# gyhandy/Neural-Sim-NeRF

Hardware: AMD Instinct MI355X
Metric: Mray-samples/sec at 400x400, 64+128 samples, 8x256 MLP (higher is better)
Workload: dtype f16x2

## Files before the change

### neural_sim_nerf_amd/csrc/nsr_kernels.hip

```cpp
#include <hip/hip_runtime.h>
#include <stdint.h>
#include "nsr_device.h"

#if !defined(NSR_UNIT_F32) && !defined(NSR_UNIT_H2) && !defined(NSR_UNIT_B3) && !defined(NSR_UNIT_X16)
#define NSR_UNIT_F32 1
#define NSR_UNIT_H2 1
#define NSR_UNIT_B3 1
#define NSR_UNIT_X16 1
#endif
#ifndef NSR_UNIT_F32
#define NSR_UNIT_F32 0
#endif
#ifndef NSR_UNIT_H2
#define NSR_UNIT_H2 0
#endif
#ifndef NSR_UNIT_B3
#define NSR_UNIT_B3 0
#endif
#ifndef NSR_UNIT_X16
#define NSR_UNIT_X16 0
#endif
#define NSR_CAT_(a, b) a##b
#define NSR_CAT(a, b) NSR_CAT_(a, b)

// ... 208 lines not shown
constexpr int kMlpH2 = 2;

template <int NMO>
__device__ __forceinline__ uint4 relu_mask(const f32x16 (&acc)[NMO]) {
  unsigned w[4] = {0u, 0u, 0u, 0u};
#pragma unroll
  for (int mo = 0; mo < NMO; ++mo)
#pragma unroll
    for (int r = 0; r < 16; ++r) {
      const int on = max(__float_as_int(acc[mo][r]), 0) - 1;
      w[mo >> 1] = __builtin_amdgcn_alignbit(w[mo >> 1], (unsigned)on, 31);
    }
  return make_uint4(w[0], w[1], w[2], w[3]);
}

__device__ __forceinline__ float enc_trig(float a, int k) {
  const double kMagic = 6755399441055744.0;
  const double t = (double)a * 0.63661977236758134308;
  const double tm = t + kMagic;
  const int n = __double2loint(tm) + k;
  const double f = t - (tm - kMagic);
  const float r = (float)(f * 1.57079632679489661923);
  const float z = r * r;
  float ps = __builtin_fmaf(-1.9515295891e-4f, z, 8.3321608736e-3f);
  ps = __builtin_fmaf(ps, z, -1.6666654611e-1f);
  ps = __builtin_fmaf(ps * z, r, r);
  float pc = __builtin_fmaf(2.443315711809948e-5f, z, -1.388731625493765e-3f);
  pc = __builtin_fmaf(pc, z, 4.166664568298827e-2f);
  pc = __builtin_fmaf(pc * z, z, __builtin_fmaf(-0.5f, z, 1.0f));
  const float v = (n & 1) ? pc : ps;
  return __uint_as_float(__float_as_uint(v) ^ ((unsigned)(n & 2) << 30));
}

__device__ __forceinline__ float enc_domain(float x, int nfreq) {
  return __builtin_fabsf(x) < ldexpf(1.0f, 25 - nfreq) ? x : __builtin_nanf("");
}

__device__ __forceinline__ float enc_poison(float px, float py, float pz, float vx, float vy, float vz) {
  const float a = (enc_domain(px, kMultires) * 0.0f + enc_domain(py, kMultires) * 0.0f) + enc_domain(pz, kMultires) * 0.0f;
  const float b = (enc_domain(vx, kMultiresViews) * 0.0f + enc_domain(vy, kMultiresViews) * 0.0f) +
                  enc_domain(vz, kMultiresViews) * 0.0f;
  return __builtin_fabsf(a + b);
}

template <bool CAPTURE, int MODE = kMlpF32>
__device__ __forceinline__ void mlp_pass(Ring& rg, const float* aux, f32x4 (&A0)[4], f32x4 (&A1)[4], int lane,
                                         float px, float py, float pz, float vx, float vy, float vz,
                                         float (&raw)[4], uint4* mask_dst = nullptr , int mask_tid = 0,
                                         long long* tp = nullptr ) {
#ifdef NSR_PHASE_TIMING
  long long tpl = clock64();
#define NSR_TP(i) do { if (tp) { const long long t_ = clock64(); tp[i] += t_ - tpl; tpl = t_; } } while (0)
#else
#define NSR_TP(i) do { } while (0)
#endif
  const int h = lane >> 5;
  const int h4 = aux_half(lane);
  const float poison = enc_poison(px, py, pz, vx, vy, vz);
  float e[32];
  float ed[16];
  {
    const float p[3] = {px, py, pz};
    const float v[3] = {vx, vy, vz};
#pragma unroll
    for (int L = 0; L < kMultires; ++L)
#pragma unroll
      for (int ax = 0; ax < 3; ++ax) e[3 * L + ax] = enc_trig(enc_domain(p[ax], kMultires) * (float)(1 << L), h);
#pragma unroll
    for (int L = 0; L < kMultiresViews; ++L)
#pragma unroll
      for (int ax = 0; ax < 3; ++ax) ed[3 * L + ax] = enc_trig(enc_domain(v[ax], kMultiresViews) * (float)(1 << L), h);
    e[30] = h ? pz : px;
    e[31] = h ? 0.0f : py;
    ed[12] = h ? vz : vx;
    ed[13] = h ? 0.0f : vy;
    ed[14] = 0.0f;
    ed[15] = 0.0f;
  }

  f32x16 acc[8];
  f32x16 in[8];
  auto enc_src = [&](int kb, int i) { return e[(8 * kb + i) & 31]; };
  auto in_src = [&](int kb, int i) { return in[(kb >> 1) & 7][8 * (kb & 1) + i]; };
  constexpr bool B3 = MODE == kMlpB3;
  constexpr bool H2M = MODE == kMlpH2;
  float amax = 0.0f;
  const float* h2s = aux + kAuxH2Scale;
#if NSR_H2_SCHED == 3 && !defined(NSR_EXP_H2_NOFRAG) && !defined(NSR_EXP_H2_HALFBARRIER) && !defined(NSR_EXP_H2_NOSPLIT)
  constexpr bool TAIL = H2M && !CAPTURE;
#else
  constexpr bool TAIL = false;
#endif
  static_assert(kAuxBiasV == kAuxBias + 9 * 256, "the views layer's bias follows feature_linear's: 'bias of layer L + 1' for L = 8");
  NSR_TP(0);
  load_bias<8>(aux + kAuxBias, h4, acc);
  NSR_TP(2);
  if constexpr (B3) gemm_b3<8, 2>(rg, A0, A1, enc_src, acc, lane);
  else if constexpr (TAIL)
    gemm_h2_tail<4>(rg, A0, A1, enc_src, H2Scale{{h2s[0], 0.0f}, 4}, acc, lane, amax, H2Tail{acc, in, 0, h2_lds_base(aux + kAuxBias + 256, h4)});
  else if constexpr (H2M) gemm_h2<8, 4>(rg, A0, A1, enc_src, H2Scale{{h2s[0], 0.0f}, 4}, acc, lane, amax);
  else seg<8, 8>(rg, A0, A1, BArr<32>{e}, acc, lane);
  NSR_TP(1);
  if (CAPTURE) mask_dst[mask_tid] = relu_mask<8>(acc);
  if constexpr (!TAIL) {
#pragma unroll
    for (int mo = 0; mo < 8; ++mo) in[mo] = relu16(acc[mo]);
  }

  float alpha_part = 0.0f;
#pragma unroll 1
  for (int L = 1; L <= 8; ++L) {
    if constexpr (!TAIL) load_bias<8>(aux + kAuxBias + L * 256, h4, acc);
    NSR_TP(2);
    if (L == 5) {
      if constexpr (B3) gemm_b3<8, 2>(rg, A0, A1, enc_src, acc, lane);
      else if constexpr (H2M) gemm_h2<8, 4>(rg, A0, A1, enc_src, H2Scale{{h2s[9], 0.0f}, 4}, acc, lane, amax);
      else seg<8, 8>(rg, A0, A1, BArr<32>{e}, acc, lane);
      NSR_TP(1);
    }
    if (L == 8) {
      const float* wa = aux + kAuxWAlpha;
#pragma unroll
      for (int tq = 0; tq < 32; ++tq) {
        f32x4 w = *(const f32x4*)(wa + tq * 8 + h4);
#pragma unroll
        for (int kk = 0; kk < 4; ++kk)
          alpha_part = __builtin_fmaf(w[kk], in[(4 * tq + kk) >> 4][(4 * tq + kk) & 15], alpha_part);
      }
    }
    if constexpr (B3) gemm_b3<8, 8>(rg, A0, A1, in_src, acc, lane);
    else if constexpr (TAIL)
      gemm_h2_tail<16>(rg, A0, A1, in_src, H2Scale{{h2s[L], 0.0f}, 16}, acc, lane, amax,
                       H2Tail{acc, in, (L == 8) ? (int)0x80000000 : 0, h2_lds_base(aux + kAuxBias + (L + 1) * 256, h4)});
    else if constexpr (H2M) gemm_h2<8, 16>(rg, A0, A1, in_src, H2Scale{{h2s[L], 0.0f}, 16}, acc, lane, amax);
    else seg<8, 32>(rg, A0, A1, BRegs16<8>{in}, acc, lane);
    NSR_TP(1);
    if (CAPTURE && L < 8) mask_dst[L * 256 + mask_tid] = relu_mask<8>(acc);
    if constexpr (!TAIL) {
      const int thr = (L == 8) ? (int)0x80000000 : 0;
#pragma unroll
      for (int mo = 0; mo < 8; ++mo) in[mo] = clamp_bits16(acc[mo], thr);
    }
  }

  f32x16 av[4];
  if constexpr (TAIL) {
#pragma unroll
    for (int mo = 0; mo < 4; ++mo) av[mo] = acc[mo];
  } else {
    load_bias<4>(aux + kAuxBiasV, h4, av);
  }
  NSR_TP(2);
  if constexpr (B3) {
    auto v_src = [&](int kb, int i) {
      return kb < 16 ? in[(kb >> 1) & 7][8 * (kb & 1) + i] : (kb < 18 ? ed[(8 * (kb - 16) + i) & 15] : 0.0f);
    };
    gemm_b3<4, 5>(rg, A0, A1, v_src, av, lane);
  } else if constexpr (H2M) {
    auto v_src = [&](int kb, int i) { return kb < 16 ? in[(kb >> 1) & 7][8 * (kb & 1) + i] : ed[(8 * (kb - 16) + i) & 15]; };
    gemm_h2<4, 18>(rg, A0, A1, v_src, H2Scale{{h2s[10], h2s[11]}, 16}, av, lane, amax);
  } else {
    seg<4, 36>(rg, A0, A1, BViews{in, ed}, av, lane);
  }
  NSR_TP(1);
  if (CAPTURE) mask_dst[8 * 256 + mask_tid] = relu_mask<4>(av);

  float part[4] = {0.0f, 0.0f, 0.0f, alpha_part};
  if constexpr (H2M) {
    const float ov = amax > kH2Max ? __builtin_nanf("") : 0.0f;
    part[0] = part[1] = part[2] = ov;
    part[3] = alpha_part + ov;
  }
#pragma unroll
  for (int c = 0; c < 3; ++c) {
    const float* wr = aux + kAuxWRgb + c * 128;
#pragma unroll
    for (int mo = 0; mo < 4; ++mo)
#pragma unroll
      for (int rq = 0; rq < 4; ++rq) {
        f32x4 w = *(const f32x4*)(wr + (mo * 4 + rq) * 8 + h4);
#pragma unroll
        for (int ri = 0; ri < 4; ++ri)
          part[c] = __builtin_fmaf(w[ri], fmaxf(av[mo][rq * 4 + ri], 0.0f), part[c]);
      }
  }
#pragma unroll
  for (int c = 0; c < 4; ++c) {
    float other = __shfl_xor(part[c], 32);
    float lo_half = h ? other : part[c];
    float hi_half = h ? part[c] : other;
    raw[c] = ((lo_half + hi_half) + aux[(c < 3) ? (kAuxBRgb + c) : kAuxBAlpha]) + poison;
  }
  NSR_TP(3);
#undef NSR_TP
}

template <int NSS, int NFS>
struct ItemStateT {
  static constexpr int kNS = NSS, kNF = NFS;
  float tcoarse[NSS];
  float ufine[128];
  float ray[2][16];
  float zc[2][NSS];
  float rawc[2][NSS][4];
  float w0[2][NSS];
  float cdf[2][NSS];
  float zs[2][128];
  float zf[2][NFS];
  float rawf[2][NFS][4];
  float alpha[2][NFS];
  float wf[2][NFS];
  float tf[2][NFS];
  float om[2][NFS];
  float bwd_scratch[2][NFS][2];
  float psum[2][NFS / 32][12];
  float gnorm[2];
  float res[2][8];
};
typedef ItemStateT<64, 192> ItemState;
typedef ItemStateT<128, 256> ItemStateBig;
static_assert(sizeof(ItemState) == 23048, "the YCB-V layout is part of the shipped kernels' LDS budget");
template <int NS> struct ItemStateFor { typedef ItemState type; };
template <> struct ItemStateFor<128> { typedef ItemStateBig type; };

__device__ __forceinline__ float sigmoidf_(float x) { return 1.0f / (1.0f + expf(-x)); }

template <int S, int R = 2, int STRIDE = S, typename ST>
__device__ __forceinline__ void composite(ST& st, const float* z, float* raw, float* wout, float* tout, int tid,
                                          const float* noise = nullptr ,
                                          long long row0 = 0, int valid = R) {
  static_assert(S % 8 == 0, "scan is unrolled by 8");
  for (int idx = tid; idx < R * S; idx += 256) {
    const int r = idx / S, i = idx - r * S;
    const float* zr = z + r * STRIDE;
    float dist = (i < S - 1) ? (zr[i + 1] - zr[i]) : 1e10f;
    dist = dist * st.ray[r][11];
    float* q = raw + (r * STRIDE + i) * 4;
    if (noise) q[3] = q[3] + noise[(row0 + (r < valid ? r : 0)) * S + i];
    const float sigma = fmaxf(q[3], 0.0f);
    const float a = 1.0f - expf(-sigma * dist);
    st.alpha[r][i] = a;
    st.om[r][i] = (1.0f - a) + 1e-10f;
    q[0] = sigmoidf_(q[0]);
    q[1] = sigmoidf_(q[1]);
    q[2] = sigmoidf_(q[2]);
  }
  __syncthreads();
  if ((tid & 63) == 0 && tid < 64 * R) {
    const int r = tid >> 6;
    double T = 1.0;
#pragma unroll 1
    for (int i0 = 0; i0 < S; i0 += 8) {
      double f[8];
#pragma unroll
// ... 356 lines not shown
  unsigned ovf_cap;
  const unsigned long long* item_list;
  const unsigned* item_count;
  unsigned item_cap;
};

__device__ __forceinline__ void load_aux(char* smem, const RenderArgs& a, int tid) {
  float* dst = (float*)(smem + kLdsAux);
  for (int i = tid; i < kAuxFloats; i += 256) {
    dst[i] = a.aux[0][i];
    dst[kAuxFloats + i] = a.aux[1][i];
  }
}

#if NSR_UNIT_F32
__global__ void k_set_args(const RenderArgs a, RenderArgs* dst) {
  *dst = a;
  *a.work_counter = 0ull;
  if (a.ovf_stat) a.ovf_stat[0] = 0u;
  if (a.epoch_counter) dst->epoch = *a.epoch_counter = *a.epoch_counter % 4094u + 1u;
}
#endif

constexpr long long kItemMask = (1ll << 62) - 1;
__device__ __forceinline__ long long queue_next_item(const RenderArgs& q) {
  const unsigned long long v = atomicAdd(q.work_counter, 1ull);
  if (q.item_list) {
    unsigned n = *q.item_count;
    n = n < q.item_cap ? n : q.item_cap;
    return v < (unsigned long long)n ? (long long)q.item_list[v] : -1ll;
  }
  return v < (unsigned long long)((q.n_rays + 1) >> 1) ? (long long)(v | (3ull << 62)) : -1ll;
}
__device__ __forceinline__ long long queue_items(const RenderArgs& q) {
  if (q.item_list) { const unsigned n = *q.item_count; return (long long)(n < q.item_cap ? n : q.item_cap); }
  return (q.n_rays + 1) >> 1;
}
__device__ __forceinline__ void range_mark(int* ovf, float chk, int lane) {
#ifndef NSR_EXP_NO_RANGE
  if (chk != chk && lane < 32) atomicAdd(ovf, 1);
#endif
}
__device__ __forceinline__ unsigned range_report(const RenderArgs& a, int* ovf, long long item, int valid) {
#ifdef NSR_EXP_NO_RANGE
  return 0u;
#endif
  const int p0 = ovf[0], p1 = valid == 2 ? ovf[1] : 0;
  if ((p0 | p1) != 0 && a.ovf_stat) {
    const unsigned long long mask = (p0 ? 1ull : 0ull) | (p1 ? 2ull : 0ull);
    const unsigned n = atomicAdd(a.ovf_stat, 1u);
    atomicAdd(a.ovf_stat + 1, (unsigned)(p0 + p1));
    if (n < a.ovf_cap) {
      a.ovf_items[n] = (unsigned long long)item | (mask << 62);
      atomicAdd(a.ovf_stat + 2, (unsigned)((p0 != 0) + (p1 != 0)));
    } else {
      atomicAdd(a.ovf_stat + 3, 1u);
      return (unsigned)mask;
    }
  }
  return 0u;
}
__device__ __forceinline__ void range_poison(const RenderArgs& a, long long ray0, unsigned mask) {
  const float qn = __builtin_nanf("");
  for (int r = 0; r < 2; ++r) {
    if (!((mask >> r) & 1u)) continue;
    const long long rr = ray0 + r;
    float* const v3[2] = {a.rgb, a.rgb0};
    float* const v1[5] = {a.disp, a.acc, a.disp0, a.acc0, a.z_std};
    for (int k = 0; k < 2; ++k) if (v3[k]) { v3[k][rr * 3] = qn; v3[k][rr * 3 + 1] = qn; v3[k][rr * 3 + 2] = qn; }
    for (int k = 0; k < 5; ++k) if (v1[k]) v1[k][rr] = qn;
  }
}

#ifdef NSR_PHASE_TIMING
#define NSR_T(i) do { if (threadIdx.x == 0) { const long long t_ = clock64(); tacc[i] += t_ - tlast; tlast = t_; } } while (0)
#else
#define NSR_T(i) do { } while (0)
#endif

template <int MODE, int NI = 128, int NS = 64>
__device__ __forceinline__ void render32_body(const RenderArgs* __restrict__ ap, char* smem) {
  constexpr bool B3 = MODE == kMlpB3;
  constexpr int NF = NS + NI;
  constexpr int NP = (2 * NF + 127) / 128;
  constexpr int NPC = (2 * NS + 127) / 128;
  constexpr int LNS = NS == 32 ? 5 : (NS == 64 ? 6 : 7);
  typedef typename ItemStateFor<NS>::type ST;
  static_assert((NS == 32 || NS == 64 || NS == 128) && NF % 32 == 0 && NS <= ST::kNS && NF <= ST::kNF,
                "a wave's points belong to one ray; the item state holds kNS coarse / kNF fine samples per ray");
  const RenderArgs& a_setup = *ap;
#ifdef NSR_PHASE_TIMING
  long long tacc[8] = {0, 0, 0, 0, 0, 0, 0, 0};
  long long tpass[4] = {0, 0, 0, 0};
  long long tlast = clock64();
#define NSR_TPASS tpass
#else
#define NSR_TPASS nullptr
#endif
  const int tid0 = threadIdx.x;
  const int lane = tid0 & 63;
  const int wave = __builtin_amdgcn_readfirstlane(tid0 >> 6);
  const int j = lane & 31;
  ST& st = *(ST*)(smem + kLdsState);

  const long long n_rays = a_setup.n_rays;
  if ((long long)blockIdx.x >= queue_items(a_setup)) return;
  const int fine = a_setup.fine;
  int* ovf = (int*)&st.ray[1][14];

  Ring rg;
  ring_init(rg, smem, a_setup.nets, a_setup.net_stride, fine ? NPC + NP : NPC, wave, lane);
  rg.pn0 = NPC; rg.pn1 = NPC + NP;

  f32x4 A0[4], A1[4];
  if constexpr (B3) ring_start<kRingSlots, kStreamSlabsB3, kStreamSlabsB3Bwd>(rg, A0, lane);
  else if constexpr (MODE == kMlpH2) ring_start<kRingSlots, kStreamSlabs, kStreamSlabs, kH2RingLag>(rg, A0, lane);
  else ring_start(rg, A0, lane);

  load_aux(smem, a_setup, tid0);
  if (tid0 < NS) st.tcoarse[tid0] = a_setup.tcoarse[tid0];
  if (tid0 < NI) st.ufine[tid0] = a_setup.ufine[tid0];
  __syncthreads();
  const float* aux_c = (const float*)(smem + kLdsAux);

  long long* item_slot = (long long*)&st.ray[0][14];
  auto next_item = [&]() -> long long {
    if (opaque_v(tid0) == 0) *item_slot = queue_next_item(*opaque_s(ap));
    __syncthreads();
    const long long v = uniform64(*item_slot);
    __syncthreads();
    return v;
  };
  long long packed = next_item();
  int pass = 0;
#pragma unroll 1
  while (packed != -1ll) {
    const long long item = packed & kItemMask;
    const long long ray0 = item * 2;
    const int valid = (ray0 + 1 < n_rays) ? 2 : 1;
    const int wmask = (int)((unsigned long long)packed >> 62) & (valid == 2 ? 3 : 1);
    auto wr = [&](int r) { return ((wmask >> r) & 1) != 0; };
    if (pass == 0) {
      const RenderArgs& a = *opaque_s(ap);
      const int tid = opaque_v(tid0);
      const float near_ = a.near_, far_ = a.far_;
      if (tid < 2) {
        const long long rr = ray0 + (tid < valid ? tid : 0);
        float o[3], d[3];
        if (a.camera) {
          const long long hw = (long long)a.H * a.W;
          const long long v = rr / hw;
          const int pix = (int)(rr - v * hw);
          gen_ray(a.c2w + v * 12, a.fx, a.fy, a.cx, a.cy, pix / a.W, pix % a.W, o, d);
        } else {
#pragma unroll
          for (int c = 0; c < 3; ++c) { o[c] = a.rays_o[rr * 3 + c]; d[c] = a.rays_d[rr * 3 + c]; }
        }
        const float nrm = sqrtf(((d[0] * d[0]) + (d[1] * d[1])) + (d[2] * d[2]));
        const float* vd = a.camera ? nullptr : a.viewdirs;
#pragma unroll
        for (int c = 0; c < 3; ++c) {
          st.ray[tid][c] = o[c]; st.ray[tid][3 + c] = d[c];
          st.ray[tid][6 + c] = vd ? vd[rr * 3 + c] : d[c] / nrm;
        }
        st.ray[tid][9] = a.near_rays ? a.near_rays[rr] : near_;
        st.ray[tid][10] = a.near_rays ? a.far_rays[rr] : far_;
        st.ray[tid][11] = nrm;
        st.ray[tid][12] = a.white_bkgd ? 1.0f : 0.0f;
      }
      if (MODE == kMlpH2 && (tid == 64 || tid == 65)) ovf[tid - 64] = 0;
      if (tid < 2 * NS) {
        const int r = tid >> LNS, i = tid & (NS - 1);
        const float t = st.tcoarse[i];
        const long long rb = ray0 + (r < valid ? r : 0);
        st.zc[r][i] = coarse_z(a.near_rays ? a.near_rays[rb] : near_, a.near_rays ? a.far_rays[rb] : far_, t, a.lindisp);
      }
      __syncthreads();
      if (a.t_rand) perturb_coarse_z<NS>(st, a.t_rand, ray0, valid, tid);
      NSR_T(0);
    }

    {
      int r, i;
      const float* zsrc;
      float* dst;
      bool real = true;
      if ((NPC == 1) ? (pass == 0) : (pass < NPC)) {
        if constexpr (NS == 64) {
          r = wave >> 1; i = 32 * (wave & 1) + j;
        } else {
          int q0 = 128 * pass + 32 * wave;
          if (2 * NS % 128 != 0 && q0 >= 2 * NS) { q0 = 2 * NS - 32; real = false; }
          r = q0 >> LNS; i = (q0 & (NS - 1)) + j;
        }
        zsrc = &st.zc[r][i]; dst = st.rawc[r][i];
      } else {
        int q0 = 128 * (pass - NPC) + 32 * wave;
        if (2 * NF % 128 != 0 && q0 >= 2 * NF) { q0 = 2 * NF - 32; real = false; }
        r = q0 / NF; i = q0 - r * NF + j;
        zsrc = &st.zf[r][i]; dst = st.rawf[r][i];
      }
      const float z = *zsrc;
      const float* ry = st.ray[r];
      float raw[4];
      mlp_pass<false, MODE>(rg, aux_c + (((NPC == 1) ? (pass == 0) : (pass < NPC)) ? 0 : kAuxFloats), A0, A1, lane, ry[0] + ry[3] * z, ry[1] + ry[4] * z,
               ry[2] + ry[5] * z, ry[6], ry[7], ry[8], raw, nullptr, 0, NSR_TPASS);
      if (lane < 32 && real) *(f32x4*)dst = f32x4{raw[0], raw[1], raw[2], raw[3]};
      if constexpr (MODE == kMlpH2) { if (real) range_mark(ovf + r, (raw[0] + raw[1]) + (raw[2] + raw[3]), lane); }
    }
    NSR_T(1);

    const RenderArgs& a = *opaque_s(ap);
    const int tid = opaque_v(tid0);
    if (NPC > 1 && pass < NPC - 1) {
      ++pass;
    } else if ((NPC == 1) ? (pass == 0) : (pass < NPC)) {
      __syncthreads();
      if (a.dbg_raw0) {
        if constexpr (NS == ST::kNS) {
          for (int idx = tid; idx < 2 * NS * 4; idx += 256) if (wr(idx >> (LNS + 2))) a.dbg_raw0[ray0 * (NS * 4) + idx] = (&st.rawc[0][0][0])[idx];
        } else {
          for (int idx = tid; idx < 2 * NS * 4; idx += 256)
            if (wr(idx >> (LNS + 2))) a.dbg_raw0[ray0 * (NS * 4) + idx] = (&st.rawc[idx >> (LNS + 2)][0][0])[idx & (NS * 4 - 1)];
        }
        __syncthreads();
      }
      composite<NS, 2, ST::kNS>(st, &st.zc[0][0], &st.rawc[0][0][0], &st.w0[0][0], &st.tf[0][0], tid, a.noise0, ray0, valid);
      if (tid < 16 && wr(tid >> 3)) {
        const int r = tid >> 3, c = tid & 7;
        const long long rr = ray0 + r;
        const float v = st.res[r][c];
        float* rgb_dst = fine ? a.rgb0 : a.rgb;
        float* disp_dst = fine ? a.disp0 : a.disp;
        float* acc_dst = fine ? a.acc0 : a.acc;
        if (c < 3) { if (rgb_dst) rgb_dst[rr * 3 + c] = v; }
        else if (c == 3) { if (disp_dst) disp_dst[rr] = v; }
        else if (c == 4) { if (acc_dst) acc_dst[rr] = v; }
      }
      if (a.dbg_w0)
        for (int idx = tid; idx < 2 * NS; idx += 256)
          if (wr(idx >> LNS)) a.dbg_w0[ray0 * NS + idx] = NS == ST::kNS ? (&st.w0[0][0])[idx] : st.w0[idx >> LNS][idx & (NS - 1)];
      if (!fine) {
        if (MODE == kMlpH2 && tid == 0) { if (const unsigned m = range_report(a, ovf, item, valid)) range_poison(a, ray0, m); }
        __syncthreads();
        if constexpr (NPC > 1) pass = 0;
        packed = next_item(); continue;
      }
      NSR_T(2);

#ifdef NSR_PHASE_TIMING
      int64_t* inds = nullptr;
#else
      int64_t* inds = (int64_t*)a.dbg_inds;
#endif
      sample_pdf_item<2, NI, NS>(st, st.ufine, &st.w0[0][1], ST::kNS,
                             [&](int r, int k) { return 0.5f * (st.zc[r][k + 1] + st.zc[r][k]); },
                             inds ? inds + ray0 * NI : nullptr, NI, tid, valid, a.u_rays, ray0, wmask);
      NSR_T(3);
      if (wave < 2) {
        const float sd = zstd_wave<NI>(st, wave, lane);
        if (lane == 0 && wr(wave) && a.z_std) a.z_std[ray0 + wave] = sd;
      }
      if (a.dbg_zs)
        for (int idx = tid; idx < 2 * 128; idx += 256)
          if (wr(idx >> 7) && (idx & 127) < NI) a.dbg_zs[(ray0 + (idx >> 7)) * NI + (idx & 127)] = (&st.zs[0][0])[idx];
      NSR_T(4);
      merge_sort_item<2, NI, NS>(st, tid);
      if (a.dbg_zf)
        for (int idx = tid; idx < 2 * ST::kNF; idx += 256)
          if (wr(idx / ST::kNF) && idx % ST::kNF < NF) a.dbg_zf[(ray0 + idx / ST::kNF) * NF + idx % ST::kNF] = (&st.zf[0][0])[idx];
      NSR_T(5);
      pass = NPC;
    } else if (pass < NPC + NP - 1) {
      ++pass;
    } else {
      __syncthreads();
      if (a.dbg_raw) {
        for (int idx = tid; idx < 2 * ST::kNF * 4; idx += 256)
          if (wr(idx / (ST::kNF * 4)) && idx % (ST::kNF * 4) < NF * 4)
            a.dbg_raw[(ray0 + idx / (ST::kNF * 4)) * (NF * 4) + idx % (ST::kNF * 4)] = (&st.rawf[0][0][0])[idx];
        __syncthreads();
      }
      composite<NF, 2, ST::kNF>(st, &st.zf[0][0], &st.rawf[0][0][0], &st.wf[0][0], &st.tf[0][0], tid, a.noise1, ray0, valid);
      if (tid < 16 && wr(tid >> 3)) {
        const int r = tid >> 3, c = tid & 7;
        const long long rr = ray0 + r;
        const float v = st.res[r][c];
        if (c < 3) { if (a.rgb) a.rgb[rr * 3 + c] = v; }
        else if (c == 3) { if (a.disp) a.disp[rr] = v; }
        else if (c == 4) { if (a.acc) a.acc[rr] = v; }
      }
      if (MODE == kMlpH2 && tid == 0) { if (const unsigned m = range_report(a, ovf, item, valid)) range_poison(a, ray0, m); }
      __syncthreads();
      NSR_T(6);
      pass = 0;
      packed = next_item();
    }
  }
  asm volatile("s_waitcnt vmcnt(0)" ::: "memory");
#ifdef NSR_PHASE_TIMING
  if (tid0 == 0 && a_setup.dbg_raw == nullptr && a_setup.dbg_inds)
    for (int i = 0; i < 8; ++i) a_setup.dbg_inds[blockIdx.x * 8 + i] = tacc[i];
  if (tid0 == 0 && a_setup.dbg_raw == nullptr && a_setup.dbg_inds)
    for (int i = 0; i < 4; ++i) a_setup.dbg_inds[(long long)gridDim.x * 8 + blockIdx.x * 4 + i] = tpass[i];
#endif
#undef NSR_TPASS
}

#define NSR_RENDER_KERNEL_1(NAME, ...)                                                               \
  __global__ void __launch_bounds__(256, 1) NAME(const RenderArgs* __restrict__ ap) {                \
    extern __shared__ __attribute__((aligned(16))) char smem[];                                      \
    render32_body<__VA_ARGS__>(ap, smem);                                                            \
  }
#define NSR_RENDER_KERNEL_0(NAME, ...) __global__ void __launch_bounds__(256, 1) NAME(const RenderArgs* __restrict__ ap);
#define NSR_RENDER_KERNEL(UNIT, NAME, ...) NSR_CAT(NSR_RENDER_KERNEL_, UNIT)(NAME, __VA_ARGS__)
NSR_RENDER_KERNEL(NSR_UNIT_F32, k_render, kMlpF32)
NSR_RENDER_KERNEL(NSR_UNIT_B3, k_render_b3, kMlpB3)
NSR_RENDER_KERNEL(NSR_UNIT_H2, k_render_h2, kMlpH2)
NSR_RENDER_KERNEL(NSR_UNIT_H2, k_render_h2_n64, kMlpH2, 64)
NSR_RENDER_KERNEL(NSR_UNIT_H2, k_render_h2_n32, kMlpH2, 32)
NSR_RENDER_KERNEL(NSR_UNIT_B3, k_render_b3_n64, kMlpB3, 64)
NSR_RENDER_KERNEL(NSR_UNIT_B3, k_render_b3_n32, kMlpB3, 32)
NSR_RENDER_KERNEL(NSR_UNIT_H2, k_render_h2_n96, kMlpH2, 96, 64)
NSR_RENDER_KERNEL(NSR_UNIT_B3, k_render_b3_n96, kMlpB3, 96, 64)
NSR_RENDER_KERNEL(NSR_UNIT_H2, k_render_h2_c32_n64, kMlpH2, 64, 32)
NSR_RENDER_KERNEL(NSR_UNIT_B3, k_render_b3_c32_n64, kMlpB3, 64, 32)
NSR_RENDER_KERNEL(NSR_UNIT_H2, k_render_h2_c128_n128, kMlpH2, 128, 128)
NSR_RENDER_KERNEL(NSR_UNIT_B3, k_render_b3_c128_n128, kMlpB3, 128, 128)
#undef NSR_RENDER_KERNEL
#undef NSR_RENDER_KERNEL_0
#undef NSR_RENDER_KERNEL_1

__device__ __forceinline__ f32x16 apply_mask(f32x16 x, unsigned word, int shift) {
  f32x16 r;
#pragma unroll
// ... 1811 lines not shown
```

Before: 283.0.

## Share sin/cos evaluation and precompute per-ray view encodings in LDS

On the H2 tail path, positional encoding now computes sine and cosine together from a single range reduction, with each lane-half computing different frequency bands and exchanging results through permlane32_swap. This roughly halves the trig work per sample. View-direction encodings are now computed once per ray by 48 threads into an LDS area that shares storage with psum, and each sample reads them back as float4s instead of recomputing. The first-layer bias load also switches to the tail's LDS loader. Risks include the union with psum aliasing live data, and a possible race because no barrier follows the dir_enc writes before the MLP reads them.

```diff
diff --git a/neural_sim_nerf_amd/csrc/nsr_kernels.hip b/neural_sim_nerf_amd/csrc/nsr_kernels.hip
--- a/neural_sim_nerf_amd/csrc/nsr_kernels.hip
+++ b/neural_sim_nerf_amd/csrc/nsr_kernels.hip
@@ -264,6 +264,25 @@
   return __uint_as_float(__float_as_uint(v) ^ ((unsigned)(n & 2) << 30));
 }
 
+__device__ __forceinline__ void enc_trig2(float a, float& s, float& c) {
+  const double kMagic = 6755399441055744.0;
+  const double t = (double)a * 0.63661977236758134308;
+  const double tm = t + kMagic;
+  const int n = __double2loint(tm);
+  const double f = t - (tm - kMagic);
+  const float r = (float)(f * 1.57079632679489661923);
+  const float z = r * r;
+  float ps = __builtin_fmaf(-1.9515295891e-4f, z, 8.3321608736e-3f);
+  ps = __builtin_fmaf(ps, z, -1.6666654611e-1f);
+  ps = __builtin_fmaf(ps * z, r, r);
+  float pc = __builtin_fmaf(2.443315711809948e-5f, z, -1.388731625493765e-3f);
+  pc = __builtin_fmaf(pc, z, 4.166664568298827e-2f);
+  pc = __builtin_fmaf(pc * z, z, __builtin_fmaf(-0.5f, z, 1.0f));
+  const int n1 = n + 1;
+  s = __uint_as_float(__float_as_uint((n & 1) ? pc : ps) ^ ((unsigned)(n & 2) << 30));
+  c = __uint_as_float(__float_as_uint((n1 & 1) ? pc : ps) ^ ((unsigned)(n1 & 2) << 30));
+}
+
 __device__ __forceinline__ float enc_domain(float x, int nfreq) {
   return __builtin_fabsf(x) < ldexpf(1.0f, 25 - nfreq) ? x : __builtin_nanf("");
 }
@@ -279,7 +298,8 @@
 __device__ __forceinline__ void mlp_pass(Ring& rg, const float* aux, f32x4 (&A0)[4], f32x4 (&A1)[4], int lane,
                                          float px, float py, float pz, float vx, float vy, float vz,
                                          float (&raw)[4], uint4* mask_dst = nullptr , int mask_tid = 0,
-                                         long long* tp = nullptr ) {
+                                         long long* tp = nullptr ,
+                                         const float* ed_lds = nullptr ) {
 #ifdef NSR_PHASE_TIMING
   long long tpl = clock64();
 #define NSR_TP(i) do { if (tp) { const long long t_ = clock64(); tp[i] += t_ - tpl; tpl = t_; } } while (0)
@@ -289,19 +309,41 @@
   const int h = lane >> 5;
   const int h4 = aux_half(lane);
   const float poison = enc_poison(px, py, pz, vx, vy, vz);
+  constexpr bool H2M = MODE == kMlpH2;
+#if NSR_H2_SCHED == 3 && !defined(NSR_EXP_H2_NOFRAG) && !defined(NSR_EXP_H2_HALFBARRIER) && !defined(NSR_EXP_H2_NOSPLIT)
+  constexpr bool TAIL = H2M && !CAPTURE;
+#else
+  constexpr bool TAIL = false;
+#endif
+  constexpr bool POS_ONCE = TAIL, DIR_ONCE = TAIL;
   float e[32];
   float ed[16];
   {
     const float p[3] = {px, py, pz};
     const float v[3] = {vx, vy, vz};
-#pragma unroll
-    for (int L = 0; L < kMultires; ++L)
-#pragma unroll
-      for (int ax = 0; ax < 3; ++ax) e[3 * L + ax] = enc_trig(enc_domain(p[ax], kMultires) * (float)(1 << L), h);
-#pragma unroll
-    for (int L = 0; L < kMultiresViews; ++L)
-#pragma unroll
-      for (int ax = 0; ax < 3; ++ax) ed[3 * L + ax] = enc_trig(enc_domain(v[ax], kMultiresViews) * (float)(1 << L), h);
+    if constexpr (POS_ONCE) {
+      const float pd[3] = {enc_domain(px, kMultires), enc_domain(py, kMultires), enc_domain(pz, kMultires)};
+      const float base = h ? 32.0f : 1.0f;
+#pragma unroll
+      for (int k = 0; k < 15; ++k) {
+        float sn, cs;
+        enc_trig2(pd[k % 3] * ((float)(1 << (k / 3)) * base), sn, cs);
+        const auto sw = __builtin_amdgcn_permlane32_swap(__float_as_uint(sn), __float_as_uint(cs), false, false);
+        e[k] = __uint_as_float(sw[0]);
+        e[15 + k] = __uint_as_float(sw[1]);
+      }
+    } else {
+#pragma unroll
+      for (int L = 0; L < kMultires; ++L)
+#pragma unroll
+        for (int ax = 0; ax < 3; ++ax) e[3 * L + ax] = enc_trig(enc_domain(p[ax], kMultires) * (float)(1 << L), h);
+    }
+    if constexpr (!DIR_ONCE) {
+#pragma unroll
+      for (int L = 0; L < kMultiresViews; ++L)
+#pragma unroll
+        for (int ax = 0; ax < 3; ++ax) ed[3 * L + ax] = enc_trig(enc_domain(v[ax], kMultiresViews) * (float)(1 << L), h);
+    }
     e[30] = h ? pz : px;
     e[31] = h ? 0.0f : py;
     ed[12] = h ? vz : vx;
@@ -315,17 +357,17 @@
   auto enc_src = [&](int kb, int i) { return e[(8 * kb + i) & 31]; };
   auto in_src = [&](int kb, int i) { return in[(kb >> 1) & 7][8 * (kb & 1) + i]; };
   constexpr bool B3 = MODE == kMlpB3;
-  constexpr bool H2M = MODE == kMlpH2;
   float amax = 0.0f;
   const float* h2s = aux + kAuxH2Scale;
-#if NSR_H2_SCHED == 3 && !defined(NSR_EXP_H2_NOFRAG) && !defined(NSR_EXP_H2_HALFBARRIER) && !defined(NSR_EXP_H2_NOSPLIT)
-  constexpr bool TAIL = H2M && !CAPTURE;
-#else
-  constexpr bool TAIL = false;
-#endif
   static_assert(kAuxBiasV == kAuxBias + 9 * 256, "the views layer's bias follows feature_linear's: 'bias of layer L + 1' for L = 8");
   NSR_TP(0);
-  load_bias<8>(aux + kAuxBias, h4, acc);
+  if constexpr (POS_ONCE) {
+    const H2Tail t0{acc, in, 0, h2_lds_base(aux + kAuxBias, h4)};
+#pragma unroll
+    for (int k = 0; k < 8; ++k) { t0.load(k, 0); t0.load(k, 1); t0.load(k, 2); t0.load(k, 3); }
+  } else {
+    load_bias<8>(aux + kAuxBias, h4, acc);
+  }
   NSR_TP(2);
   if constexpr (B3) gemm_b3<8, 2>(rg, A0, A1, enc_src, acc, lane);
   else if constexpr (TAIL)
@@ -389,6 +431,13 @@
     };
     gemm_b3<4, 5>(rg, A0, A1, v_src, av, lane);
   } else if constexpr (H2M) {
+    if constexpr (DIR_ONCE) {
+#pragma unroll
+      for (int q = 0; q < 3; ++q) {
+        const f32x4 w = *(const f32x4*)(ed_lds + 4 * q);
+        ed[4 * q + 0] = w[0]; ed[4 * q + 1] = w[1]; ed[4 * q + 2] = w[2]; ed[4 * q + 3] = w[3];
+      }
+    }
     auto v_src = [&](int kb, int i) { return kb < 16 ? in[(kb >> 1) & 7][8 * (kb & 1) + i] : ed[(8 * (kb - 16) + i) & 15]; };
     gemm_h2<4, 18>(rg, A0, A1, v_src, H2Scale{{h2s[10], h2s[11]}, 16}, av, lane, amax);
   } else {
@@ -445,13 +494,18 @@
   float tf[2][NFS];
   float om[2][NFS];
   float bwd_scratch[2][NFS][2];
-  float psum[2][NFS / 32][12];
+  union {
+    float psum[2][NFS / 32][12];
+    float dir_enc[2][2][12];
+  };
   float gnorm[2];
   float res[2][8];
 };
 typedef ItemStateT<64, 192> ItemState;
 typedef ItemStateT<128, 256> ItemStateBig;
 static_assert(sizeof(ItemState) == 23048, "the YCB-V layout is part of the shipped kernels' LDS budget");
+static_assert(offsetof(ItemState, dir_enc) % 16 == 0 && offsetof(ItemStateBig, dir_enc) % 16 == 0 && kLdsState % 16 == 0 &&
+              sizeof(ItemState::dir_enc) <= sizeof(ItemState::psum), "dir_enc rows are read as three float4");
 template <int NS> struct ItemStateFor { typedef ItemState type; };
 template <> struct ItemStateFor<128> { typedef ItemStateBig type; };
 
@@ -1018,6 +1072,10 @@
         st.zc[r][i] = coarse_z(a.near_rays ? a.near_rays[rb] : near_, a.near_rays ? a.far_rays[rb] : far_, t, a.lindisp);
       }
       __syncthreads();
+      if (MODE == kMlpH2 && tid >= 256 - 48) {
+        const int t = tid - (256 - 48), r = t / 24, hh = (t / 12) & 1, k = t % 12;
+        st.dir_enc[r][hh][k] = enc_trig(enc_domain(st.ray[r][6 + k % 3], kMultiresViews) * (float)(1 << (k / 3)), hh);
+      }
       if (a.t_rand) perturb_coarse_z<NS>(st, a.t_rand, ray0, valid, tid);
       NSR_T(0);
     }
@@ -1046,7 +1104,7 @@
       const float* ry = st.ray[r];
       float raw[4];
       mlp_pass<false, MODE>(rg, aux_c + (((NPC == 1) ? (pass == 0) : (pass < NPC)) ? 0 : kAuxFloats), A0, A1, lane, ry[0] + ry[3] * z, ry[1] + ry[4] * z,
-               ry[2] + ry[5] * z, ry[6], ry[7], ry[8], raw, nullptr, 0, NSR_TPASS);
+               ry[2] + ry[5] * z, ry[6], ry[7], ry[8], raw, nullptr, 0, NSR_TPASS, st.dir_enc[NSR_IDX(r, 2)][lane >> 5]);
       if (lane < 32 && real) *(f32x4*)dst = f32x4{raw[0], raw[1], raw[2], raw[3]};
       if constexpr (MODE == kMlpH2) { if (real) range_mark(ovf + r, (raw[0] + raw[1]) + (raw[2] + raw[3]), lane); }
     }
```

Result: no change. 285.7 (median of 6 runs) (+1.0%).

## Overlap fine compositing of previous item with coarse stage via double-buffered ray state

Applied to the files above, without the earlier changes.

Restructures the persistent render loop so the fine-pass compositing of the previous ray pair runs on waves 2-3 while waves 0-1 do coarse compositing, PDF sampling and merge for the current pair. Ray and fine-z state are double-buffered in the backward scratch area, and the next queue item is prefetched with a ticket taken during the coarse stage. Per-ray work becomes wave-local (composite_wave, sample_pdf_wave, merge_wave) using wave barriers, and __syncthreads is replaced by a lighter lgkmcnt+s_barrier. This removes block-wide barriers and serial phases per item, at the cost of more LDS aliasing complexity, serial lane-0 double-precision scans, and the risk of scratch-overlap bugs.

```diff
diff --git a/neural_sim_nerf_amd/csrc/nsr_kernels.hip b/neural_sim_nerf_amd/csrc/nsr_kernels.hip
--- a/neural_sim_nerf_amd/csrc/nsr_kernels.hip
+++ b/neural_sim_nerf_amd/csrc/nsr_kernels.hip
@@ -874,6 +874,14 @@
   }
   return v < (unsigned long long)((q.n_rays + 1) >> 1) ? (long long)(v | (3ull << 62)) : -1ll;
 }
+__device__ __forceinline__ long long queue_item_of(const RenderArgs& q, unsigned long long v) {
+  if (q.item_list) {
+    unsigned n = *q.item_count;
+    n = n < q.item_cap ? n : q.item_cap;
+    return v < (unsigned long long)n ? (long long)q.item_list[v] : -1ll;
+  }
+  return v < (unsigned long long)((q.n_rays + 1) >> 1) ? (long long)(v | (3ull << 62)) : -1ll;
+}
 __device__ __forceinline__ long long queue_items(const RenderArgs& q) {
   if (q.item_list) { const unsigned n = *q.item_count; return (long long)(n < q.item_cap ? n : q.item_cap); }
   return (q.n_rays + 1) >> 1;
@@ -912,6 +920,241 @@
     for (int k = 0; k < 2; ++k) if (v3[k]) { v3[k][rr * 3] = qn; v3[k][rr * 3 + 1] = qn; v3[k][rr * 3 + 2] = qn; }
     for (int k = 0; k < 5; ++k) if (v1[k]) v1[k][rr] = qn;
   }
+}
+
+__device__ __forceinline__ void wave_lds_sync() {
+  __builtin_amdgcn_fence(__ATOMIC_RELEASE, "wavefront");
+  __builtin_amdgcn_wave_barrier();
+  __builtin_amdgcn_fence(__ATOMIC_ACQUIRE, "wavefront");
+}
+__device__ __forceinline__ void lds_barrier() { asm volatile("s_waitcnt lgkmcnt(0)\n\ts_barrier" ::: "memory"); }
+
+template <typename ST>
+struct FwdItemExtra {
+  float om[2][ST::kNS];
+  float tf[2][ST::kNS];
+  float zf[2][ST::kNF];
+  float ray[2][16];
+  float res[2][8];
+  long long pend;
+  long long next;
+};
+
+template <int S>
+__device__ __forceinline__ void composite_wave(const float* ry, const float* zr, float* q, float* wr, float* tr, float* omr,
+                                               int lane, const float* noise ,
+                                               float (&res)[6]) {
+  static_assert(S % 8 == 0, "scan is unrolled by 8");
+  constexpr int K = (S + 63) / 64;
+  float al[K];
+#pragma unroll
+  for (int k = 0; k < K; ++k) {
+    const int i = lane + 64 * k;
+    al[k] = 0.0f;
+    if (i < S) {
+      float dist = (i < S - 1) ? (zr[i + 1] - zr[i]) : 1e10f;
+      dist = dist * ry[11];
+      if (noise) q[i * 4 + 3] = q[i * 4 + 3] + noise[i];
+      const float sigma = fmaxf(q[i * 4 + 3], 0.0f);
+      const float a = 1.0f - expf(-sigma * dist);
+      al[k] = a;
+      omr[i] = (1.0f - a) + 1e-10f;
+      q[i * 4 + 0] = sigmoidf_(q[i * 4 + 0]);
+      q[i * 4 + 1] = sigmoidf_(q[i * 4 + 1]);
+      q[i * 4 + 2] = sigmoidf_(q[i * 4 + 2]);
+    }
+  }
+  wave_lds_sync();
+  if (lane == 0) {
+    double T = 1.0;
+#pragma unroll 1
+    for (int i0 = 0; i0 < S; i0 += 8) {
+      double f[8];
+#pragma unroll
+      for (int k = 0; k < 8; ++k) f[k] = (double)omr[i0 + k];
+#pragma unroll
+      for (int k = 0; k < 8; ++k) {
+        tr[i0 + k] = (float)T;
+        T = T * f[k];
+      }
+    }
+  }
+  wave_lds_sync();
+  float cr = 0.f, cg = 0.f, cb = 0.f, depth = 0.f, acc = 0.f;
+#pragma unroll
+  for (int k = 0; k < K; ++k) {
+    const int i = lane + 64 * k;
+    if (i < S) {
+      const float w = al[k] * tr[i];
+      wr[i] = w;
+      cr = cr + w * q[i * 4 + 0];
+      cg = cg + w * q[i * 4 + 1];
+      cb = cb + w * q[i * 4 + 2];
+      depth = depth + w * zr[i];
+      acc = acc + w;
+    }
+  }
+#pragma unroll
+  for (int m = 32; m >= 1; m >>= 1) {
+    cr += __shfl_xor(cr, m); cg += __shfl_xor(cg, m); cb += __shfl_xor(cb, m);
+    depth += __shfl_xor(depth, m); acc += __shfl_xor(acc, m);
+  }
+  const float qd = depth / acc;
+  float disp;
+  if (qd != qd) disp = qd;
+  else disp = 1.0f / fmaxf(1e-10f, qd);
+  if (ry[12] != 0.0f) {
+    const float bg = 1.0f - acc;
+    cr = cr + bg; cg = cg + bg; cb = cb + bg;
+  }
+  res[0] = cr; res[1] = cg; res[2] = cb; res[3] = disp; res[4] = acc; res[5] = depth;
+  wave_lds_sync();
+}
+
+template <int NI, int NS>
+__device__ __forceinline__ void sample_pdf_wave(const float* w, const float* zc, float* x, float* pdf, float* cdf, float* zs,
+                                                const float* u ,
+                                                int64_t* inds_out , int lane) {
+  constexpr int NW = NS - 2, NC = NS - 1;
+  constexpr int NVEC = NW / 8, SILP = NVEC / 4;
+  constexpr int KW = (NW + 63) / 64;
+  float xv[KW];
+#pragma unroll
+  for (int k = 0; k < KW; ++k) {
+    const int i = lane + 64 * k;
+    xv[k] = 0.0f;
+    if (i < NW) { xv[k] = w[i] + 1e-5f; x[i] = xv[k]; }
+  }
+  wave_lds_sync();
+  const int j = lane & 7;
+  float lj;
+  if constexpr (NS == 64) {
+    const float p0 = ((x[j] + x[32 + j]) + x[40 + j]) + x[48 + j];
+    lj = ((p0 + x[8 + j]) + x[16 + j]) + x[24 + j];
+  } else {
+    float ps[4] = {0.0f, 0.0f, 0.0f, 0.0f};
+#pragma unroll
+    for (int i = 0; i < SILP; ++i)
+#pragma unroll
+      for (int k = 0; k < 4; ++k) ps[k] = ps[k] + x[(i * 4 + k) * 8 + j];
+#pragma unroll
+    for (int v = SILP * 4; v < NVEC; ++v) ps[0] = ps[0] + x[v * 8 + j];
+    lj = ((ps[0] + ps[1]) + ps[2]) + ps[3];
+  }
+  float total = 0.0f;
+#pragma unroll
+  for (int i = NVEC * 8; i < NW; ++i) total = total + x[i];
+#pragma unroll
+  for (int jj = 0; jj < 8; ++jj) total = total + __shfl(lj, jj);
+#pragma unroll
+  for (int k = 0; k < KW; ++k) {
+    const int i = lane + 64 * k;
+    if (i < NW) pdf[i] = xv[k] / total;
+  }
+  wave_lds_sync();
+  if (lane == 0) {
+    double run = 0.0;
+    cdf[0] = 0.0f;
+#pragma unroll 1
+    for (int i0 = 0; i0 < NVEC * 8; i0 += 8) {
+      double f[8];
+#pragma unroll
+      for (int k = 0; k < 8; ++k) f[k] = (double)pdf[i0 + k];
+#pragma unroll
+      for (int k = 0; k < 8; ++k) { run = run + f[k]; cdf[i0 + k + 1] = (float)run; }
+    }
+#pragma unroll
+    for (int i = NVEC * 8; i < NW; ++i) { run = run + (double)pdf[i]; cdf[i + 1] = (float)run; }
+  }
+  wave_lds_sync();
+#pragma unroll
+  for (int kk = 0; kk < (NI + 63) / 64; ++kk) {
+    const int k = lane + 64 * kk;
+    if (k < NI) {
+      const float uu = u[k];
+      int lo = 0, hi = NC;
+      while (lo < hi) {
+        const int mid = (lo + hi) >> 1;
+        if (cdf[NSR_IDX(mid, NC)] <= uu) lo = mid + 1; else hi = mid;
+      }
+      const int ind = lo;
+      const int below = NSR_IDX(max(ind - 1, 0), NC);
+      const int above = NSR_IDX(min(ind, NC - 1), NC);
+      const float c0 = cdf[below], c1 = cdf[above];
+      const float b0 = 0.5f * (zc[below + 1] + zc[below]), b1 = 0.5f * (zc[above + 1] + zc[above]);
+      float denom = c1 - c0;
+      if (denom < 1e-5f) denom = 1.0f;
+      const float t = (uu - c0) / denom;
+      zs[NSR_IDX(k, 128)] = b0 + t * (b1 - b0);
+      if (inds_out) inds_out[k] = (int64_t)ind;
+    }
+  }
+  wave_lds_sync();
+}
+
+template <int NI, int NS>
+__device__ __forceinline__ void merge_wave(const float* zc, const float* zs, float* zf, int lane) {
+  constexpr int NF = NS + NI;
+  constexpr bool kPow2 = (NI & (NI - 1)) == 0 && (NS & (NS - 1)) == 0;
+  constexpr int K = (NF + 63) / 64;
+  int bad = 0;
+#pragma unroll
+  for (int kk = 0; kk < K; ++kk) {
+    const int k = lane + 64 * kk;
+    if (k < NS - 1) bad |= !(zc[k] <= zc[k + 1]);
+    else if (k >= NS && k < NF - 1) bad |= !(zs[k - NS] <= zs[k - NS + 1]);
+  }
+  const bool any_bad = __builtin_amdgcn_ballot_w64(bad != 0) != 0;
+  if (!any_bad) {
+#pragma unroll
+    for (int kk = 0; kk < K; ++kk) {
+      const int k = lane + 64 * kk;
+      if (k < NS) {
+        const float x = zc[k];
+        int lb = 0;
+        if constexpr (kPow2) {
+#pragma unroll
+          for (int sft = NI / 2; sft > 0; sft >>= 1) lb += (zs[lb + sft - 1] < x) ? sft : 0;
+          lb += (zs[lb] < x) ? 1 : 0;
+        } else {
+          int hi = NI;
+          while (lb < hi) { const int mid = (lb + hi) >> 1; if (zs[NSR_IDX(mid, NI)] < x) lb = mid + 1; else hi = mid; }
+        }
+        zf[NSR_IDX(k + lb, NF)] = x;
+      } else if (k < NF) {
+        const float x = zs[k - NS];
+        int ub = 0;
+        if constexpr (kPow2) {
+#pragma unroll
+          for (int sft = NS / 2; sft > 0; sft >>= 1) ub += (zc[ub + sft - 1] <= x) ? sft : 0;
+          ub += (zc[ub] <= x) ? 1 : 0;
+        } else {
+          int hi = NS;
+          while (ub < hi) { const int mid = (ub + hi) >> 1; if (zc[NSR_IDX(mid, NS)] <= x) ub = mid + 1; else hi = mid; }
+        }
+        zf[NSR_IDX((k - NS) + ub, NF)] = x;
+      }
+    }
+  } else {
+#pragma unroll 1
+    for (int kk = 0; kk < K; ++kk) {
+      const int k = lane + 64 * kk;
+      if (k < NF) {
+        const float x = (k < NS) ? zc[k] : zs[k - NS];
+        int rank = 0;
+        for (int jx = 0; jx < NS; ++jx) {
+          const float y = zc[jx];
+          rank += (y < x) || (y == x && jx < k);
+        }
+        for (int jx = 0; jx < NI; ++jx) {
+          const float y = zs[jx];
+          rank += (y < x) || (y == x && (jx + NS) < k);
+        }
+        zf[NSR_IDX(rank, NF)] = x;
+      }
+    }
+  }
+  wave_lds_sync();
 }
 
 #ifdef NSR_PHASE_TIMING
@@ -948,7 +1191,10 @@
   const long long n_rays = a_setup.n_rays;
   if ((long long)blockIdx.x >= queue_items(a_setup)) return;
   const int fine = a_setup.fine;
-  int* ovf = (int*)&st.ray[1][14];
+  typedef FwdItemExtra<ST> XT;
+  static_assert(offsetof(ST, res) - offsetof(ST, bwd_scratch) >= sizeof(XT) && offsetof(ST, bwd_scratch) % 8 == 0 &&
+                offsetof(XT, pend) % 8 == 0, "the forward scratch lives in the item state's backward scratch");
+  XT& xs = *(XT*)&st.bwd_scratch[0][0][0];
 
   Ring rg;
   ring_init(rg, smem, a_setup.nets, a_setup.net_stride, fine ? NPC + NP : NPC, wave, lane);
@@ -962,19 +1208,63 @@
   load_aux(smem, a_setup, tid0);
   if (tid0 < NS) st.tcoarse[tid0] = a_setup.tcoarse[tid0];
   if (tid0 < NI) st.ufine[tid0] = a_setup.ufine[tid0];
+  if (tid0 == 0) xs.pend = -1ll;
   __syncthreads();
   const float* aux_c = (const float*)(smem + kLdsAux);
 
   long long* item_slot = (long long*)&st.ray[0][14];
   auto next_item = [&]() -> long long {
     if (opaque_v(tid0) == 0) *item_slot = queue_next_item(*opaque_s(ap));
-    __syncthreads();
+    lds_barrier();
     const long long v = uniform64(*item_slot);
-    __syncthreads();
+    lds_barrier();
     return v;
   };
+
+  auto fine_wave = [&](long long pk, int pp, int r) {
+    const RenderArgs& a = *opaque_s(ap);
+    const long long ray0 = (pk & kItemMask) * 2;
+    const int valid = (ray0 + 1 < n_rays) ? 2 : 1;
+    const int wmask = (int)((unsigned long long)pk >> 62) & (valid == 2 ? 3 : 1);
+    const float* ry = pp ? xs.ray[r] : st.ray[r];
+    const float* zr = pp ? xs.zf[r] : st.zf[r];
+    float* q = &st.rawf[r][0][0];
+    if (a.dbg_raw && ((wmask >> r) & 1)) {
+      for (int idx = lane; idx < NF * 4; idx += 64) a.dbg_raw[(ray0 + r) * (NF * 4) + idx] = q[idx];
+      wave_lds_sync();
+    }
+    float res[6];
+    composite_wave<NF>(ry, zr, q, st.wf[r], st.tf[r], st.om[r], lane,
+                       a.noise1 ? a.noise1 + (ray0 + (r < valid ? r : 0)) * NF : nullptr, res);
+    if (lane == 0) {
+#pragma unroll
+      for (int c = 0; c < 6; ++c) st.res[r][c] = res[c];
+    }
+  };
+  auto fine_out = [&](long long pk, int pp) {
+    const RenderArgs& a = *opaque_s(ap);
+    const int tid = opaque_v(tid0);
+    const long long item = pk & kItemMask;
+    const long long ray0 = item * 2;
+    const int valid = (ray0 + 1 < n_rays) ? 2 : 1;
+    const int wmask = (int)((unsigned long long)pk >> 62) & (valid == 2 ? 3 : 1);
+    if (tid < 16 && ((wmask >> (tid >> 3)) & 1)) {
+      const int r = tid >> 3, c = tid & 7;
+      const long long rr = ray0 + r;
+      const float v = st.res[r][c];
+      if (c < 3) { if (a.rgb) a.rgb[rr * 3 + c] = v; }
+      else if (c == 3) { if (a.disp) a.disp[rr] = v; }
+      else if (c == 4) { if (a.acc) a.acc[rr] = v; }
+    }
+    if (MODE == kMlpH2 && tid == 0) {
+      int* povf = (int*)(pp ? &xs.ray[1][14] : &st.ray[1][14]);
+      if (const unsigned m = range_report(a, povf, item, valid)) range_poison(a, ray0, m);
+    }
+  };
+
   long long packed = next_item();
   int pass = 0;
+  int par = 0;
 #pragma unroll 1
   while (packed != -1ll) {
     const long long item = packed & kItemMask;
@@ -982,6 +1272,9 @@
     const int valid = (ray0 + 1 < n_rays) ? 2 : 1;
     const int wmask = (int)((unsigned long long)packed >> 62) & (valid == 2 ? 3 : 1);
     auto wr = [&](int r) { return ((wmask >> r) & 1) != 0; };
+    float (*const ray)[16] = par ? xs.ray : st.ray;
+    float* const zf = par ? &xs.zf[0][0] : &st.zf[0][0];
+    int* const ovf = (int*)&ray[1][14];
     if (pass == 0) {
       const RenderArgs& a = *opaque_s(ap);
       const int tid = opaque_v(tid0);
@@ -1002,13 +1295,13 @@
         const float* vd = a.camera ? nullptr : a.viewdirs;
 #pragma unroll
         for (int c = 0; c < 3; ++c) {
-          st.ray[tid][c] = o[c]; st.ray[tid][3 + c] = d[c];
-          st.ray[tid][6 + c] = vd ? vd[rr * 3 + c] : d[c] / nrm;
-        }
-        st.ray[tid][9] = a.near_rays ? a.near_rays[rr] : near_;
-        st.ray[tid][10] = a.near_rays ? a.far_rays[rr] : far_;
-        st.ray[tid][11] = nrm;
-        st.ray[tid][12] = a.white_bkgd ? 1.0f : 0.0f;
+          ray[tid][c] = o[c]; ray[tid][3 + c] = d[c];
+          ray[tid][6 + c] = vd ? vd[rr * 3 + c] : d[c] / nrm;
+        }
+        ray[tid][9] = a.near_rays ? a.near_rays[rr] : near_;
+        ray[tid][10] = a.near_rays ? a.far_rays[rr] : far_;
+        ray[tid][11] = nrm;
+        ray[tid][12] = a.white_bkgd ? 1.0f : 0.0f;
       }
       if (MODE == kMlpH2 && (tid == 64 || tid == 65)) ovf[tid - 64] = 0;
       if (tid < 2 * NS) {
@@ -1017,7 +1310,7 @@
         const long long rb = ray0 + (r < valid ? r : 0);
         st.zc[r][i] = coarse_z(a.near_rays ? a.near_rays[rb] : near_, a.near_rays ? a.far_rays[rb] : far_, t, a.lindisp);
       }
-      __syncthreads();
+      lds_barrier();
       if (a.t_rand) perturb_coarse_z<NS>(st, a.t_rand, ray0, valid, tid);
       NSR_T(0);
     }
@@ -1040,10 +1333,10 @@
         int q0 = 128 * (pass - NPC) + 32 * wave;
         if (2 * NF % 128 != 0 && q0 >= 2 * NF) { q0 = 2 * NF - 32; real = false; }
         r = q0 / NF; i = q0 - r * NF + j;
-        zsrc = &st.zf[r][i]; dst = st.rawf[r][i];
+        zsrc = &zf[r * ST::kNF + i]; dst = st.rawf[r][i];
       }
       const float z = *zsrc;
-      const float* ry = st.ray[r];
+      const float* ry = ray[r];
       float raw[4];
       mlp_pass<false, MODE>(rg, aux_c + (((NPC == 1) ? (pass == 0) : (pass < NPC)) ? 0 : kAuxFloats), A0, A1, lane, ry[0] + ry[3] * z, ry[1] + ry[4] * z,
                ry[2] + ry[5] * z, ry[6], ry[7], ry[8], raw, nullptr, 0, NSR_TPASS);
@@ -1057,21 +1350,64 @@
     if (NPC > 1 && pass < NPC - 1) {
       ++pass;
     } else if ((NPC == 1) ? (pass == 0) : (pass < NPC)) {
-      __syncthreads();
-      if (a.dbg_raw0) {
-        if constexpr (NS == ST::kNS) {
-          for (int idx = tid; idx < 2 * NS * 4; idx += 256) if (wr(idx >> (LNS + 2))) a.dbg_raw0[ray0 * (NS * 4) + idx] = (&st.rawc[0][0][0])[idx];
-        } else {
-          for (int idx = tid; idx < 2 * NS * 4; idx += 256)
-            if (wr(idx >> (LNS + 2))) a.dbg_raw0[ray0 * (NS * 4) + idx] = (&st.rawc[idx >> (LNS + 2)][0][0])[idx & (NS * 4 - 1)];
-        }
-        __syncthreads();
-      }
-      composite<NS, 2, ST::kNS>(st, &st.zc[0][0], &st.rawc[0][0][0], &st.w0[0][0], &st.tf[0][0], tid, a.noise0, ray0, valid);
+      lds_barrier();
+      const long long pend = fine ? uniform64(xs.pend) : -1ll;
+      const bool puller = fine && tid == 192;
+      unsigned long long ticket = 0ull;
+      if (puller) ticket = atomicAdd(a.work_counter, 1ull);
+      if (wave < 2) {
+        const int r = wave;
+        float* q = &st.rawc[r][0][0];
+        if (a.dbg_raw0 && wr(r)) {
+          for (int idx = lane; idx < NS * 4; idx += 64) a.dbg_raw0[(ray0 + r) * (NS * 4) + idx] = q[idx];
+          wave_lds_sync();
+        }
+        float res[6];
+        composite_wave<NS>(ray[r], st.zc[r], q, st.w0[r], xs.tf[r], xs.om[r], lane,
+                           a.noise0 ? a.noise0 + (ray0 + (r < valid ? r : 0)) * NS : nullptr, res);
+        if (lane == 0) {
+#pragma unroll
+          for (int c = 0; c < 6; ++c) xs.res[r][c] = res[c];
+        }
+        if (a.dbg_w0 && wr(r))
+          for (int idx = lane; idx < NS; idx += 64) a.dbg_w0[(ray0 + r) * NS + idx] = st.w0[r][idx];
+        NSR_T(2);
+        if (fine) {
+#ifdef NSR_PHASE_TIMING
+          int64_t* inds = nullptr;
+#else
+          int64_t* inds = (int64_t*)a.dbg_inds;
+#endif
+          sample_pdf_wave<NI, NS>(&st.w0[r][1], st.zc[r], xs.tf[r], xs.om[r], st.cdf[r], st.zs[r],
+                                  a.u_rays ? a.u_rays + (ray0 + (r < valid ? r : 0)) * 128 : st.ufine,
+                                  (inds && wr(r)) ? inds + (ray0 + r) * NI : nullptr, lane);
+          NSR_T(3);
+          const float sd = zstd_wave<NI>(st, r, lane);
+          if (lane == 0 && wr(r) && a.z_std) a.z_std[ray0 + r] = sd;
+          if (a.dbg_zs && wr(r))
+            for (int k = lane; k < NI; k += 64) a.dbg_zs[(ray0 + r) * NI + k] = st.zs[r][k];
+          NSR_T(4);
+          merge_wave<NI, NS>(st.zc[r], st.zs[r], zf + r * ST::kNF, lane);
+          if (a.dbg_zf && wr(r))
+            for (int k = lane; k < NF; k += 64) a.dbg_zf[(ray0 + r) * NF + k] = zf[r * ST::kNF + k];
+          NSR_T(5);
+        }
+      } else if (pend != -1ll) {
+#ifdef NSR_PHASE_TIMING
+        const long long t0_ = clock64();
+#endif
+        fine_wave(pend, par ^ 1, wave - 2);
+#ifdef NSR_PHASE_TIMING
+        if (threadIdx.x == 128) tacc[7] += clock64() - t0_;
+#endif
+      }
+      if (puller) xs.next = queue_item_of(a, ticket);
+      lds_barrier();
+      if (pend != -1ll) fine_out(pend, par ^ 1);
       if (tid < 16 && wr(tid >> 3)) {
         const int r = tid >> 3, c = tid & 7;
         const long long rr = ray0 + r;
-        const float v = st.res[r][c];
+        const float v = xs.res[r][c];
         float* rgb_dst = fine ? a.rgb0 : a.rgb;
         float* disp_dst = fine ? a.disp0 : a.disp;
         float* acc_dst = fine ? a.acc0 : a.acc;
@@ -1079,70 +1415,37 @@
         else if (c == 3) { if (disp_dst) disp_dst[rr] = v; }
         else if (c == 4) { if (acc_dst) acc_dst[rr] = v; }
       }
-      if (a.dbg_w0)
-        for (int idx = tid; idx < 2 * NS; idx += 256)
-          if (wr(idx >> LNS)) a.dbg_w0[ray0 * NS + idx] = NS == ST::kNS ? (&st.w0[0][0])[idx] : st.w0[idx >> LNS][idx & (NS - 1)];
+      NSR_T(6);
       if (!fine) {
         if (MODE == kMlpH2 && tid == 0) { if (const unsigned m = range_report(a, ovf, item, valid)) range_poison(a, ray0, m); }
-        __syncthreads();
         if constexpr (NPC > 1) pass = 0;
         packed = next_item(); continue;
       }
-      NSR_T(2);
-
-#ifdef NSR_PHASE_TIMING
-      int64_t* inds = nullptr;
-#else
-      int64_t* inds = (int64_t*)a.dbg_inds;
-#endif
-      sample_pdf_item<2, NI, NS>(st, st.ufine, &st.w0[0][1], ST::kNS,
-                             [&](int r, int k) { return 0.5f * (st.zc[r][k + 1] + st.zc[r][k]); },
-                             inds ? inds + ray0 * NI : nullptr, NI, tid, valid, a.u_rays, ray0, wmask);
-      NSR_T(3);
-      if (wave < 2) {
-        const float sd = zstd_wave<NI>(st, wave, lane);
-        if (lane == 0 && wr(wave) && a.z_std) a.z_std[ray0 + wave] = sd;
-      }
-      if (a.dbg_zs)
-        for (int idx = tid; idx < 2 * 128; idx += 256)
-          if (wr(idx >> 7) && (idx & 127) < NI) a.dbg_zs[(ray0 + (idx >> 7)) * NI + (idx & 127)] = (&st.zs[0][0])[idx];
-      NSR_T(4);
-      merge_sort_item<2, NI, NS>(st, tid);
-      if (a.dbg_zf)
-        for (int idx = tid; idx < 2 * ST::kNF; idx += 256)
-          if (wr(idx / ST::kNF) && idx % ST::kNF < NF) a.dbg_zf[(ray0 + idx / ST::kNF) * NF + idx % ST::kNF] = (&st.zf[0][0])[idx];
-      NSR_T(5);
       pass = NPC;
     } else if (pass < NPC + NP - 1) {
       ++pass;
     } else {
-      __syncthreads();
-      if (a.dbg_raw) {
-        for (int idx = tid; idx < 2 * ST::kNF * 4; idx += 256)
-          if (wr(idx / (ST::kNF * 4)) && idx % (ST::kNF * 4) < NF * 4)
-            a.dbg_raw[(ray0 + idx / (ST::kNF * 4)) * (NF * 4) + idx % (ST::kNF * 4)] = (&st.rawf[0][0][0])[idx];
-        __syncthreads();
-      }
-      composite<NF, 2, ST::kNF>(st, &st.zf[0][0], &st.rawf[0][0][0], &st.wf[0][0], &st.tf[0][0], tid, a.noise1, ray0, valid);
-      if (tid < 16 && wr(tid >> 3)) {
-        const int r = tid >> 3, c = tid & 7;
-        const long long rr = ray0 + r;
-        const float v = st.res[r][c];
-        if (c < 3) { if (a.rgb) a.rgb[rr * 3 + c] = v; }
-        else if (c == 3) { if (a.disp) a.disp[rr] = v; }
-        else if (c == 4) { if (a.acc) a.acc[rr] = v; }
-      }
-      if (MODE == kMlpH2 && tid == 0) { if (const unsigned m = range_report(a, ovf, item, valid)) range_poison(a, ray0, m); }
-      __syncthreads();
-      NSR_T(6);
+      if (tid == 0) xs.pend = packed;
       pass = 0;
-      packed = next_item();
-    }
+      par ^= 1;
+      packed = uniform64(xs.next);
+    }
+  }
+  if (fine) {
+    lds_barrier();
+    const long long pend = uniform64(xs.pend);
+    if (pend != -1ll) {
+      if (wave < 2) fine_wave(pend, par ^ 1, wave);
+      lds_barrier();
+      fine_out(pend, par ^ 1);
+    }
+    NSR_T(6);
   }
   asm volatile("s_waitcnt vmcnt(0)" ::: "memory");
 #ifdef NSR_PHASE_TIMING
+  if (tid0 == 128 && a_setup.dbg_raw == nullptr && a_setup.dbg_inds) a_setup.dbg_inds[blockIdx.x * 8 + 7] = tacc[7];
   if (tid0 == 0 && a_setup.dbg_raw == nullptr && a_setup.dbg_inds)
-    for (int i = 0; i < 8; ++i) a_setup.dbg_inds[blockIdx.x * 8 + i] = tacc[i];
+    for (int i = 0; i < 7; ++i) a_setup.dbg_inds[blockIdx.x * 8 + i] = tacc[i];
   if (tid0 == 0 && a_setup.dbg_raw == nullptr && a_setup.dbg_inds)
     for (int i = 0; i < 4; ++i) a_setup.dbg_inds[(long long)gridDim.x * 8 + blockIdx.x * 4 + i] = tpass[i];
 #endif
```

After: 283.2 before, 288.4 after, median of 6. 1.02x the previous value.
